# KMASAHIRO/AVR

Hardware: AMD Instinct MI355X
Metric: ray-samples/sec/GPU (1024 rays×256 samp×512 freq) + IR render ms/pose (higher is better)
Workload: dtype f32; 1 GPU; c2_meshrir_1024x256x512; mode=pose, rays=1024, samples=256, T=1022, freq_bins=512, distinct_poses=16, parallelism=poses x1 (no data-path collective)

## Files before the change

avr_amd/csrc/hashgrid.hip:

```cpp
#include "common.h"

#include <algorithm>

using namespace avr;

namespace {

constexpr int kMaxLevels = 32;

struct LevelTable {
    int64_t offset[kMaxLevels + 1];
    float scale[kMaxLevels];
    uint32_t res[kMaxLevels];
};

__device__ __forceinline__ uint32_t grid_index(uint32_t size, uint32_t res, uint32_t x, uint32_t y,
                                               uint32_t z) {
    uint64_t stride = 1;
    uint32_t index = 0;
    const uint32_t c[3] = {x, y, z};
#pragma unroll
    for (int d = 0; d < 3; ++d) {
        if (stride > size) break;
        index += c[d] * (uint32_t)stride;
        stride *= res;
    }
    if (size < stride) index = (x * 1u) ^ (y * 2654435761u) ^ (z * 805459861u);
    return index % size;
}

template <typename Tp>
__device__ __forceinline__ float2 load_pair(const Tp* params, int64_t entry);
template <>
__device__ __forceinline__ float2 load_pair<float>(const float* params, int64_t entry) {
    return *reinterpret_cast<const float2*>(params + 2 * entry);
}
template <>
__device__ __forceinline__ float2 load_pair<__half>(const __half* params, int64_t entry) {
    return __half22float2(*reinterpret_cast<const __half2*>(params + 2 * entry));
}

template <typename Tp>
struct CornerAcc;
template <>
struct CornerAcc<float> {
    using raw = float2;
    float2 a = make_float2(0.0f, 0.0f);
    __device__ __forceinline__ static raw load(const float* table, uint32_t e) {
        return *reinterpret_cast<const float2*>(table + 2 * (size_t)e);
    }
    __device__ __forceinline__ void add(float w, raw v) {
        a.x = fmaf(w, v.x, a.x);
        a.y = fmaf(w, v.y, a.y);
    }
    __device__ __forceinline__ float2 get() const { return a; }
};
template <>
struct CornerAcc<__half> {
    using raw = __half2;
    __half2 a = __float2half2_rn(0.0f);
    __device__ __forceinline__ static raw load(const __half* table, uint32_t e) {
        return *reinterpret_cast<const __half2*>(table + 2 * (size_t)e);
    }
    __device__ __forceinline__ void add(float w, raw v) {
        const __half2 w2 = __float2half2_rn(w);
        uint32_t r, wu, vu, au;
        __builtin_memcpy(&wu, &w2, 4);
        __builtin_memcpy(&vu, &v, 4);
        __builtin_memcpy(&au, &a, 4);
        asm("v_pk_fma_f16 %0, %1, %2, %3" : "=v"(r) : "v"(wu), "v"(vu), "v"(au));
        __builtin_memcpy(&a, &r, 4);
    }
    __device__ __forceinline__ float2 get() const { return __half22float2(a); }
};

template <typename To>
__device__ __forceinline__ void store_pair(To* out, int64_t i, float2 v);
template <>
__device__ __forceinline__ void store_pair<float>(float* out, int64_t i, float2 v) {
    *reinterpret_cast<float2*>(out + 2 * i) = v;
}
template <>
__device__ __forceinline__ void store_pair<__half>(__half* out, int64_t i, float2 v) {
    *reinterpret_cast<__half2*>(out + 2 * i) = __floats2half2_rn(v.x, v.y);
}

constexpr int64_t kLevelMajorMinPoints = 16384;
inline int64_t lm_min_points() { return kLevelMajorMinPoints; }

inline bool group_loads() { return true; }

struct Corner {
    float pos[3];
    uint32_t grid[3];
};

__device__ __forceinline__ Corner locate(const float* x, float scale) {
    Corner c;
#pragma unroll
    for (int d = 0; d < 3; ++d) {
        const float p = fmaf(scale, x[d], 0.5f);
        const float fl = floorf(p);
        c.grid[d] = (uint32_t)(int)fl;
        c.pos[d] = p - fl;
    }
    return c;
}

template <typename Tp, typename To>
__global__ __launch_bounds__(256) void hashgrid_fwd_kernel(int64_t N, int L,
                                                           const float* __restrict__ x,
                                                           const Tp* __restrict__ params,
                                                           LevelTable lt, To* __restrict__ out) {
    const int64_t q = (int64_t)blockIdx.x * blockDim.x + threadIdx.x;
    if (q >= N * L) return;
    const int64_t i = q / L;
    const int l = (int)(q % L);
    const float xi[3] = {x[i * 3 + 0], x[i * 3 + 1], x[i * 3 + 2]};
    const Corner c = locate(xi, lt.scale[l]);
    const uint32_t size = (uint32_t)(lt.offset[l + 1] - lt.offset[l]);
    const uint32_t res = lt.res[l];
    const Tp* table = params + 2 * lt.offset[l];
    CornerAcc<Tp> acc;
#pragma unroll
    for (int k = 0; k < 8; ++k) {
        float wgt = 1.0f;
        uint32_t g[3];
#pragma unroll
        for (int d = 0; d < 3; ++d) {
            if (k & (1 << d)) {
                wgt *= c.pos[d];
                g[d] = c.grid[d] + 1;
            } else {
                wgt *= 1.0f - c.pos[d];
                g[d] = c.grid[d];
            }
        }
        acc.add(wgt, CornerAcc<Tp>::load(table, grid_index(size, res, g[0], g[1], g[2])));
    }
    store_pair(out, q, acc.get());
}

template <typename Tp>
struct EntryGroup;
template <>
struct EntryGroup<__half> {
    static constexpr uint32_t kN = 4;
    uint32_t d[4];
    __device__ __forceinline__ void load(const __half* table, uint32_t e) {
        const uint4 v = *reinterpret_cast<const uint4*>(table + 2 * (e & ~(kN - 1)));
        d[0] = v.x;
        d[1] = v.y;
        d[2] = v.z;
        d[3] = v.w;
    }
    __device__ __forceinline__ __half2 get(uint32_t e) const {
        const uint32_t j = e & (kN - 1);
        const uint32_t v = j == 0 ? d[0] : j == 1 ? d[1] : j == 2 ? d[2] : d[3];
        __half2 h;
        __builtin_memcpy(&h, &v, 4);
        return h;
    }
};

template <typename Tp, typename To, bool ROW_MAJOR = false, bool GROUP = false>
__global__ __launch_bounds__(256) void hashgrid_fwd_lm_kernel(int64_t N, const float* __restrict__ x,
                                                              const Tp* __restrict__ params,
                                                              LevelTable lt, To* __restrict__ out, int unit) {
    const int l = blockIdx.y;
    const int64_t i = (int64_t)blockIdx.x * 256 + threadIdx.x;
    if (i >= N) return;
    float xi[3] = {x[i * 3 + 0], x[i * 3 + 1], x[i * 3 + 2]};
    if (unit) {
#pragma unroll
        for (int d = 0; d < 3; ++d) xi[d] = 0.5f + 0.5f * xi[d];
    }
    const Corner c = locate(xi, lt.scale[l]);
    const uint32_t size = (uint32_t)(lt.offset[l + 1] - lt.offset[l]);
    const uint32_t res = lt.res[l];
    const Tp* table = params + 2 * lt.offset[l];
    CornerAcc<Tp> acc;
    float wgt[8];
    uint32_t ent[8];
#pragma unroll
    for (int k = 0; k < 8; ++k) {
        float w = 1.0f;
        uint32_t g[3];
#pragma unroll
        for (int d = 0; d < 3; ++d) {
            if (k & (1 << d)) {
                w *= c.pos[d];
                g[d] = c.grid[d] + 1;
            } else {
                w *= 1.0f - c.pos[d];
                g[d] = c.grid[d];
            }
        }
        wgt[k] = w;
        ent[k] = grid_index(size, res, g[0], g[1], g[2]);
    }
    if constexpr (GROUP) {
        constexpr uint32_t kN = EntryGroup<Tp>::kN;
        EntryGroup<Tp> grp[4];
#pragma unroll
        for (int j = 0; j < 4; ++j) grp[j].load(table, ent[2 * j]);
        using raw = typename CornerAcc<Tp>::raw;
        raw far[4];
#pragma unroll
        for (int j = 0; j < 4; ++j) {
            far[j] = grp[j].get(ent[2 * j]);
            if ((ent[2 * j + 1] ^ ent[2 * j]) >= kN) far[j] = CornerAcc<Tp>::load(table, ent[2 * j + 1]);
        }
#pragma unroll
        for (int j = 0; j < 4; ++j) {
            const raw v0 = grp[j].get(ent[2 * j]);
            const raw v1 = ((ent[2 * j + 1] ^ ent[2 * j]) >= kN) ? far[j] : grp[j].get(ent[2 * j + 1]);
            acc.add(wgt[2 * j], v0);
            acc.add(wgt[2 * j + 1], v1);
        }
    } else {
#pragma unroll
        for (int k = 0; k < 8; ++k) acc.add(wgt[k], CornerAcc<Tp>::load(table, ent[k]));
    }
    store_pair(out, ROW_MAJOR ? i * (int64_t)gridDim.y + l : (int64_t)l * N + i, acc.get());
}

template <typename Tg, int RUN>
__global__ __launch_bounds__(256) void hashgrid_bwd_kernel(int64_t N, int L, int l0,
                                                           const float* __restrict__ x,
                                                           const Tg* __restrict__ gout,
                                                           LevelTable lt,
                                                           float* __restrict__ gparams) {
    const int l = l0 + (int)blockIdx.y;
    const int slot = threadIdx.x & 15;
    const int k = slot >> 1, f = slot & 1;
    const int64_t first = ((int64_t)blockIdx.x * 16 + (threadIdx.x >> 4)) * RUN;
    const uint32_t size = (uint32_t)(lt.offset[l + 1] - lt.offset[l]);
    const uint32_t res = lt.res[l];
    const float scale = lt.scale[l];
    float* __restrict__ table = gparams + 2 * lt.offset[l];
    float xi[RUN][3], g[RUN];
#pragma unroll
    for (int it = 0; it < RUN; ++it) {
        const int64_t i = first + it;
        const int64_t ic = i < N ? i : N - 1;
#pragma unroll
        for (int d = 0; d < 3; ++d) xi[it][d] = x[ic * 3 + d];
        g[it] = i < N ? load_f(gout, ic * (2 * L) + 2 * l + f) : 0.0f;
    }
    uint32_t pe = 0xffffffffu;
    float pv = 0.0f;
#pragma unroll
    for (int it = 0; it < RUN; ++it) {
        const Corner c = locate(xi[it], scale);
        float wgt = 1.0f;
        uint32_t gg[3];
#pragma unroll
        for (int d = 0; d < 3; ++d) {
            if (k & (1 << d)) {
                wgt *= c.pos[d];
                gg[d] = c.grid[d] + 1;
            } else {
                wgt *= 1.0f - c.pos[d];
                gg[d] = c.grid[d];
            }
        }
        const uint32_t e = 2u * grid_index(size, res, gg[0], gg[1], gg[2]) + (uint32_t)f;
        const float v = wgt * g[it];
        if (e == pe) {
            pv += v;
        } else {
            if (pv != 0.0f) atomicAdd(table + pe, pv);
            pe = e;
            pv = v;
        }
    }
    if (pv != 0.0f) atomicAdd(table + pe, pv);
}

inline int bwd_run() { return 16; }

template <typename Tg>
void launch_bwd(hipStream_t st, int64_t N, int L, const float* x, const Tg* gout, const LevelTable& lt,
                float* gparams) {
    const int run = bwd_run();
    const int64_t pts_per_block = 16 * (int64_t)run;
    const dim3 grid((unsigned)((N + pts_per_block - 1) / pts_per_block), (unsigned)L);
#define AVR_HG_BWD(I)                                                                                          \
    if (run == I) {                                                                                            \
        hipLaunchKernelGGL((hashgrid_bwd_kernel<Tg, I>), grid, dim3(256), 0, st, N, L, 0, x, gout, lt, gparams); \
        return;                                                                                                \
    }
    AVR_HG_BWD(1) AVR_HG_BWD(4) AVR_HG_BWD(8) AVR_HG_BWD(16) AVR_HG_BWD(32)
#undef AVR_HG_BWD
}

int make_table(int L, const int64_t* off, const float* scale, const int32_t* res, LevelTable* lt) {
    if (L < 1 || L > kMaxLevels) return fail(AVR_E_ARG, "hashgrid: n_levels out of range (1..32)");
    for (int l = 0; l <= L; ++l) lt->offset[l] = off[l];
    for (int l = 0; l < L; ++l) {
        lt->scale[l] = scale[l];
        lt->res[l] = (uint32_t)res[l];
        if (off[l + 1] <= off[l]) return fail(AVR_E_ARG, "hashgrid: empty level");
    }
    return 0;
}

template <typename Tp, typename To, bool ROW_MAJOR>
void launch_lm(dim3 grid, hipStream_t st, int64_t N, const float* x, const void* params, LevelTable lt,
               void* out, bool grp, int unit) {
    if constexpr (std::is_same_v<Tp, __half>) {
        if (grp) {
            hipLaunchKernelGGL((hashgrid_fwd_lm_kernel<Tp, To, ROW_MAJOR, true>), grid, dim3(256), 0, st, N,
                               x, (const Tp*)params, lt, (To*)out, unit);
            return;
        }
    }
    hipLaunchKernelGGL((hashgrid_fwd_lm_kernel<Tp, To, ROW_MAJOR, false>), grid, dim3(256), 0, st, N, x,
                           (const Tp*)params, lt, (To*)out, unit);
}

template <bool ROW_MAJOR>
int launch_fwd_lm(dim3 grid, hipStream_t st, int64_t N, const float* x, const void* params,
                  int32_t param_dtype, const LevelTable& lt, void* out, int32_t out_dtype, int unit = 0) {
    const bool grp = group_loads() && ((uintptr_t)params & 15) == 0;
    if (param_dtype == AVR_DTYPE_F32 && out_dtype == AVR_DTYPE_F32)
        launch_lm<float, float, ROW_MAJOR>(grid, st, N, x, params, lt, out, grp, unit);
    else if (param_dtype == AVR_DTYPE_F32 && out_dtype == AVR_DTYPE_F16)
        launch_lm<float, __half, ROW_MAJOR>(grid, st, N, x, params, lt, out, grp, unit);
    else if (param_dtype == AVR_DTYPE_F16 && out_dtype == AVR_DTYPE_F16)
        launch_lm<__half, __half, ROW_MAJOR>(grid, st, N, x, params, lt, out, grp, unit);
    else if (param_dtype == AVR_DTYPE_F16 && out_dtype == AVR_DTYPE_F32)
        launch_lm<__half, float, ROW_MAJOR>(grid, st, N, x, params, lt, out, grp, unit);
    else
        return fail(AVR_E_ARG, "avr_hashgrid_fwd: unknown dtype");
    return 0;
}

constexpr int kPartBits = 10;
constexpr int kPartEntries = 1 << kPartBits;
constexpr int kBwdGroups = 32;
constexpr int kBwdRun = 16;
constexpr int kChunkPts = kBwdGroups * kBwdRun;
constexpr int kReduceWaves = 4;
constexpr int kMaxScatterParts = 4096;

struct BwdPlan {
    int pbase[kMaxLevels + 1];
    int nchunks;
    int max_parts;
    int slice_cap[kMaxLevels];
    int hot_above[kMaxLevels];
};

__device__ __forceinline__ void corner_value(const float (&xi)[3], float g0, float g1, int k, float scale,
                                             uint32_t size, uint32_t res, uint32_t& e, float& v0, float& v1) {
    const Corner c = locate(xi, scale);
    float wgt = 1.0f;
    uint32_t gg[3];
#pragma unroll
    for (int d = 0; d < 3; ++d) {
        if (k & (1 << d)) {
            wgt *= c.pos[d];
            gg[d] = c.grid[d] + 1;
        } else {
            wgt *= 1.0f - c.pos[d];
            gg[d] = c.grid[d];
        }
    }
    e = grid_index(size, res, gg[0], gg[1], gg[2]);
    v0 = wgt * g0;
    v1 = wgt * g1;
}

__device__ __forceinline__ int64_t glm_index(int64_t i, int64_t N, int l) { return ((int64_t)l * N + i) * 2; }

template <typename Tg>
__device__ __forceinline__ void point_inputs(int64_t i, int64_t N, int L, int l, const float* __restrict__ x,
                                             const Tg* __restrict__ glm, float (&xi)[3], float& g0, float& g1) {
    const bool live = i < N;
    const int64_t ic = live ? i : N - 1;
#pragma unroll
    for (int d = 0; d < 3; ++d) xi[d] = x[ic * 3 + d];
    const int64_t gi = glm_index(ic, N, l);
    g0 = live ? load_f(glm, gi) : 0.0f;
    g1 = live ? load_f(glm, gi + 1) : 0.0f;
}

template <typename Tg>
__global__ __launch_bounds__(256) void hg_level_major_kernel(int64_t N, int L, const Tg* __restrict__ in,
                                                             Tg* __restrict__ out) {
    extern __shared__ __attribute__((aligned(16))) char lm_s[];
    Tg* t = reinterpret_cast<Tg*>(lm_s);
    const int64_t i0 = (int64_t)blockIdx.x * 64;
    const int np = (int)min((int64_t)64, N - i0);
    const int W = 2 * L;
    for (int j = threadIdx.x; j < np * W; j += 256) t[j] = in[i0 * W + j];
    __syncthreads();
    for (int j = threadIdx.x; j < L * np * 2; j += 256) {
        const int l = j / (np * 2), r = j - l * (np * 2);
        out[((int64_t)l * N + i0) * 2 + r] = t[(r >> 1) * W + 2 * l + (r & 1)];
    }
}

template <typename Tg, class Emit>
__device__ __forceinline__ void bwd_walk(int64_t N, int L, int l, const float* __restrict__ x,
                                         const Tg* __restrict__ gout, const LevelTable& lt, Emit&& emit) {
    const int k = threadIdx.x & 7;
    const int64_t first = ((int64_t)blockIdx.x * kBwdGroups + (threadIdx.x >> 3)) * kBwdRun;
    const uint32_t size = (uint32_t)(lt.offset[l + 1] - lt.offset[l]);
    const uint32_t res = lt.res[l];
    const float scale = lt.scale[l];
    float xi[kBwdRun][3], g0[kBwdRun], g1[kBwdRun];
#pragma unroll
    for (int it = 0; it < kBwdRun; ++it) point_inputs(first + it, N, L, l, x, gout, xi[it], g0[it], g1[it]);
    uint32_t pe = 0xffffffffu;
    float p0 = 0.0f, p1 = 0.0f;
#pragma unroll
    for (int it = 0; it < kBwdRun; ++it) {
        uint32_t e;
        float v0, v1;
        corner_value(xi[it], g0[it], g1[it], k, scale, size, res, e, v0, v1);
        if (e == pe) {
            p0 += v0;
            p1 += v1;
        } else {
            if (pe != 0xffffffffu && (p0 != 0.0f || p1 != 0.0f)) emit(pe, p0, p1);
            pe = e;
            p0 = v0;
            p1 = v1;
        }
    }
    if (pe != 0xffffffffu && (p0 != 0.0f || p1 != 0.0f)) emit(pe, p0, p1);
}

template <typename Tg>
__global__ __launch_bounds__(256) void hg_bwd_count_kernel(int64_t N, int L, const float* __restrict__ x,
                                                           const Tg* __restrict__ gout, LevelTable lt,
                                                           BwdPlan plan, int* __restrict__ counts) {
    extern __shared__ int cnt_l[];
    const int l = blockIdx.y;
    const int P = plan.pbase[l + 1] - plan.pbase[l];
    for (int p = threadIdx.x; p < P; p += 256) cnt_l[p] = 0;
    __syncthreads();
    bwd_walk(N, L, l, x, gout, lt,
             [&](uint32_t e, float, float) { atomicAdd(&cnt_l[e >> kPartBits], 1); });
    __syncthreads();
    for (int p = threadIdx.x; p < P; p += 256)
        counts[(int64_t)(plan.pbase[l] + p) * plan.nchunks + blockIdx.x] = cnt_l[p];
}

__global__ __launch_bounds__(1024) void hg_bwd_scan_kernel(int total_parts, int nchunks, int* __restrict__ counts,
                                                           int* __restrict__ totals) {
    const int lane = threadIdx.x & 63;
    const int p = blockIdx.x * 16 + (threadIdx.x >> 6);
    if (p >= total_parts) return;
    int* c = counts + (int64_t)p * nchunks;
    int carry = 0;
    for (int c0 = 0; c0 < nchunks; c0 += 64) {
        const int v = c0 + lane < nchunks ? c[c0 + lane] : 0;
        int incl = v;
#pragma unroll
        for (int off = 1; off < 64; off <<= 1) {
            const int o = __shfl_up(incl, off, 64);
            if (lane >= off) incl += o;
        }
        if (c0 + lane < nchunks) c[c0 + lane] = carry + incl - v;
        carry += __shfl(incl, 63, 64);
    }
    if (lane == 0) totals[p] = carry;
}

constexpr int kDenseSlice = 1024;
constexpr int kTagRounds = 4;
constexpr int kHashedSlice = 16384;

__global__ __launch_bounds__(1024) void hg_bwd_plan_kernel(int total_parts, BwdPlan plan,
                                                           const int* __restrict__ totals,
                                                           int* __restrict__ part_start,
                                                           int* __restrict__ slice_base) {
    __shared__ int ws_t[16], ws_s[16];
    __shared__ int pbase_s[kMaxLevels + 1], hot_s[kMaxLevels], cap_s[kMaxLevels];
    const int lane = threadIdx.x & 63, wave = threadIdx.x >> 6;
    if (threadIdx.x <= kMaxLevels) pbase_s[threadIdx.x] = plan.pbase[threadIdx.x];
    if (threadIdx.x < kMaxLevels) {
        hot_s[threadIdx.x] = plan.hot_above[threadIdx.x];
        cap_s[threadIdx.x] = plan.slice_cap[threadIdx.x];
    }
    __syncthreads();
    const int per = (total_parts + 1 + 1023) / 1024;
    const int q0 = threadIdx.x * per;
    int l0 = 0;
    while (l0 < kMaxLevels && pbase_s[l0 + 1] <= q0) ++l0;
    auto slices = [&](int t, int l) {
        const int cap = t > hot_s[l] ? kDenseSlice : cap_s[l];
        return max(1, (t + cap - 1) / cap);
    };
    int st = 0, ss = 0;
    int l = l0;
    for (int j0 = 0; j0 < per; j0 += 8) {
        int tv[8];
#pragma unroll
        for (int u = 0; u < 8; ++u) {
            const int q = q0 + j0 + u;
            tv[u] = (j0 + u < per && q < total_parts) ? totals[q] : -1;
        }
#pragma unroll
        for (int u = 0; u < 8; ++u) {
            if (tv[u] < 0) break;
            const int q = q0 + j0 + u;
            while (pbase_s[l + 1] <= q) ++l;
            st += tv[u];
            ss += slices(tv[u], l);
        }
    }
    int it = st, is = ss;
#pragma unroll
    for (int off = 1; off < 64; off <<= 1) {
        const int ut = __shfl_up(it, off, 64), us = __shfl_up(is, off, 64);
        if (lane >= off) {
            it += ut;
            is += us;
        }
    }
    if (lane == 63) {
        ws_t[wave] = it;
        ws_s[wave] = is;
    }
    __syncthreads();
    int pt = 0, ps = 0;
    for (int w = 0; w < wave; ++w) {
        pt += ws_t[w];
        ps += ws_s[w];
    }
    int rt = pt + it - st, rs = ps + is - ss;
    l = l0;
    for (int j0 = 0; j0 < per; j0 += 8) {
        int tv[8];
#pragma unroll
        for (int u = 0; u < 8; ++u) {
            const int q = q0 + j0 + u;
            tv[u] = (j0 + u < per && q < total_parts) ? totals[q] : -1;
        }
#pragma unroll
        for (int u = 0; u < 8; ++u) {
            const int q = q0 + j0 + u;
            if (j0 + u >= per || q > total_parts) break;
            part_start[q] = rt;
            slice_base[q] = rs;
            if (q == total_parts) break;
            while (pbase_s[l + 1] <= q) ++l;
            rt += tv[u];
            rs += slices(tv[u], l);
        }
    }
}

constexpr int kScatMaxRecs = 256 * kBwdRun;
static_assert(((int64_t)kMaxScatterParts << kPartBits) <= (int64_t(1) << 32), "staged key: partition + entry in 32 bits");
static_assert((3 * kScatMaxRecs + 3 * kMaxScatterParts + 1) * 4 + 16 <= 160 * 1024, "scatter LDS");

template <typename Tg>
__global__ __launch_bounds__(256) void hg_bwd_scatter_kernel(int64_t N, int L, const float* __restrict__ x,
                                                             const Tg* __restrict__ gout, LevelTable lt,
                                                             BwdPlan plan, const int* __restrict__ offs,
                                                             const int* __restrict__ totals,
                                                             const int* __restrict__ part_start,
                                                             uint3* __restrict__ contrib) {
    extern __shared__ __attribute__((aligned(16))) int scat_l[];
    __shared__ int wsum[4];
    const int l = blockIdx.y;
    const int pb = plan.pbase[l];
    const int P = plan.pbase[l + 1] - pb;
    uint32_t* stage = reinterpret_cast<uint32_t*>(scat_l);
    int* base = scat_l + 3 * kScatMaxRecs;
    int* lofs = base + P;
    int* slot = lofs + P + 1;
    const int chunk = blockIdx.x, nch = plan.nchunks;
    const int lane = threadIdx.x & 63, wave = threadIdx.x >> 6;
    const int E = (P + 255) / 256;
    const int q0 = threadIdx.x * E;
    int run = 0;
    for (int j = 0; j < E; ++j) {
        const int q = q0 + j;
        if (q >= P) break;
        const int64_t at = (int64_t)(pb + q) * nch + chunk;
// ... 177 lines not shown

struct BwdLayout {
    BwdPlan plan;
    int total_parts;
    int64_t counts, totals, part_start, slice_base, glm, contrib, bytes;
    int max_slices;
    bool scatter_ok;
};

int bwd_layout(int64_t N, int L, const int64_t* off, const int32_t* res, BwdLayout* o) {
    if (L < 1 || L > kMaxLevels) return fail(AVR_E_ARG, "hashgrid: n_levels out of range (1..32)");
    BwdLayout b{};
    bool res_dense[kMaxLevels];
    for (int l = 0; l < L; ++l) {
        const double cells = res ? (double)res[l] * res[l] * res[l] : 1e300;
        res_dense[l] = cells <= (double)(off[l + 1] - off[l]);
    }
    b.plan.pbase[0] = 0;
    b.plan.max_parts = 0;
    for (int l = 0; l < L; ++l) {
        const int64_t size = off[l + 1] - off[l];
        if (size <= 0 || size % 8) return fail(AVR_E_ARG, "hashgrid: level sizes must be positive multiples of 8");
        const int64_t P = (size + kPartEntries - 1) / kPartEntries;
        if (b.plan.pbase[l] + P > (1 << 24)) return fail(AVR_E_ARG, "hashgrid: tables too large");
        b.plan.pbase[l + 1] = b.plan.pbase[l] + (int)P;
        b.plan.slice_cap[l] = res_dense[l] ? kDenseSlice : kHashedSlice;
        const double share = (double)N * 8.0 * (double)std::min<int64_t>(size, kPartEntries) / (double)size;
        b.plan.hot_above[l] = res_dense[l] ? 0 : (int)std::min(1.5 * share + 64.0, 2.0e9);
        b.plan.max_parts = std::max(b.plan.max_parts, (int)P);
    }
    const int64_t nchunks = (N + kChunkPts - 1) / kChunkPts;
    const int64_t maxc = N * L * 8;
    if (maxc >= (int64_t(1) << 31) || nchunks > 65535)
        return fail(AVR_E_ARG, "hashgrid: too many points for the partitioned backward");
    b.plan.nchunks = (int)std::max<int64_t>(nchunks, 1);
    b.total_parts = b.plan.pbase[L];
    auto al = [](int64_t v) { return (v + 255) & ~(int64_t)255; };
    int64_t o0 = 0;
    b.counts = o0;
    o0 += al((int64_t)b.total_parts * b.plan.nchunks * 4);
    b.totals = o0;
    o0 += al((int64_t)b.total_parts * 4);
    b.part_start = o0;
    o0 += al((int64_t)(b.total_parts + 1) * 4);
    b.slice_base = o0;
    o0 += al((int64_t)(b.total_parts + 1) * 4);
    b.max_slices = b.total_parts + (int)(maxc / kDenseSlice) + 1;
    b.scatter_ok = b.plan.max_parts <= kMaxScatterParts;
    b.glm = o0;
    o0 += al(N * L * 2 * 4);
    b.contrib = o0;
    o0 += al(maxc * 12);
    b.bytes = o0;
    if (b.bytes > kMaxBwdWorkspaceBytes) b.scatter_ok = false;
    *o = b;
    return 0;
}

}

extern "C" int avr_hashgrid_fwd(int64_t N, int32_t n_levels, const float* x, const void* params,
                                int32_t param_dtype, const int64_t* level_offset,
                                const float* level_scale, const int32_t* level_res, void* out,
                                int32_t out_dtype, void* stream) {
    AVR_REQUIRE(N >= 0 && x && params && level_offset && level_scale && level_res && out,
                "avr_hashgrid_fwd: bad args");
    if (N == 0) return 0;
    LevelTable lt;
    if (int e = make_table(n_levels, level_offset, level_scale, level_res, &lt)) return e;
    const int64_t work = N * n_levels;
    const dim3 grid((unsigned)((work + 255) / 256));
    hipStream_t st = as_stream(stream);
    const int L = n_levels;
    if (N >= lm_min_points()) {
        const dim3 glm((unsigned)((N + 255) / 256), (unsigned)L);
        if (int e = launch_fwd_lm<true>(glm, st, N, x, params, param_dtype, lt, out, out_dtype)) return e;
        return check_launch("avr_hashgrid_fwd");
    }
    if (param_dtype == AVR_DTYPE_F32 && out_dtype == AVR_DTYPE_F32)
        hipLaunchKernelGGL((hashgrid_fwd_kernel<float, float>), grid, dim3(256), 0, st, N, L, x,
                           (const float*)params, lt, (float*)out);
    else if (param_dtype == AVR_DTYPE_F32 && out_dtype == AVR_DTYPE_F16)
        hipLaunchKernelGGL((hashgrid_fwd_kernel<float, __half>), grid, dim3(256), 0, st, N, L, x,
                           (const float*)params, lt, (__half*)out);
    else if (param_dtype == AVR_DTYPE_F16 && out_dtype == AVR_DTYPE_F16)
        hipLaunchKernelGGL((hashgrid_fwd_kernel<__half, __half>), grid, dim3(256), 0, st, N, L, x,
                           (const __half*)params, lt, (__half*)out);
    else if (param_dtype == AVR_DTYPE_F16 && out_dtype == AVR_DTYPE_F32)
        hipLaunchKernelGGL((hashgrid_fwd_kernel<__half, float>), grid, dim3(256), 0, st, N, L, x,
                           (const __half*)params, lt, (float*)out);
    else
        return fail(AVR_E_ARG, "avr_hashgrid_fwd: unknown dtype");
    return check_launch("avr_hashgrid_fwd");
}

extern "C" int avr_hashgrid_bwd(int64_t N, int32_t n_levels, const float* x, const void* grad_out,
                                int32_t grad_dtype, const int64_t* level_offset,
                                const float* level_scale, const int32_t* level_res,
                                float* grad_params, void* stream) {
    AVR_REQUIRE(N >= 0 && x && grad_out && level_offset && level_scale && level_res && grad_params,
                "avr_hashgrid_bwd: bad args");
    if (N == 0) return 0;
    LevelTable lt;
    if (int e = make_table(n_levels, level_offset, level_scale, level_res, &lt)) return e;
    hipStream_t st = as_stream(stream);
    if (grad_dtype == AVR_DTYPE_F32)
        launch_bwd<float>(st, N, (int)n_levels, x, (const float*)grad_out, lt, grad_params);
    else if (grad_dtype == AVR_DTYPE_F16)
        launch_bwd<__half>(st, N, (int)n_levels, x, (const __half*)grad_out, lt, grad_params);
    else
        return fail(AVR_E_ARG, "avr_hashgrid_bwd: unknown grad dtype");
    return check_launch("avr_hashgrid_bwd");
}

namespace {
int fwd_lm(int64_t N, int32_t n_levels, const float* x, const void* params, int32_t param_dtype,
           const int64_t* level_offset, const float* level_scale, const int32_t* level_res, void* out,
           int32_t out_dtype, void* stream, int unit) {
    AVR_REQUIRE(N >= 0 && x && params && level_offset && level_scale && level_res && out,
                "avr_hashgrid_fwd_lm: bad args");
    if (N == 0) return 0;
    LevelTable lt;
    if (int e = make_table(n_levels, level_offset, level_scale, level_res, &lt)) return e;
    const dim3 grid((unsigned)((N + 255) / 256), (unsigned)n_levels);
    hipStream_t st = as_stream(stream);
    if (int e = launch_fwd_lm<false>(grid, st, N, x, params, param_dtype, lt, out, out_dtype, unit)) return e;
    return check_launch("avr_hashgrid_fwd_lm");
}
}

extern "C" int avr_hashgrid_fwd_lm(int64_t N, int32_t n_levels, const float* x, const void* params,
                                   int32_t param_dtype, const int64_t* level_offset,
                                   const float* level_scale, const int32_t* level_res, void* out,
                                   int32_t out_dtype, void* stream) {
    return fwd_lm(N, n_levels, x, params, param_dtype, level_offset, level_scale, level_res, out, out_dtype, stream,
                  0);
}

extern "C" int avr_hashgrid_fwd_lm_unit(int64_t N, int32_t n_levels, const float* x, const void* params,
                                        int32_t param_dtype, const int64_t* level_offset,
                                        const float* level_scale, const int32_t* level_res, void* out,
                                        int32_t out_dtype, void* stream) {
    return fwd_lm(N, n_levels, x, params, param_dtype, level_offset, level_scale, level_res, out, out_dtype, stream,
                  1);
}

namespace {

constexpr int kBiasRays = 4;

template <typename Tp>
__device__ __forceinline__ float2 encode_point_level(const float* xi, const Tp* params, const LevelTable& lt, int l) {
    const Corner c = locate(xi, lt.scale[l]);
    const uint32_t size = (uint32_t)(lt.offset[l + 1] - lt.offset[l]);
    const uint32_t res = lt.res[l];
    const Tp* table = params + 2 * lt.offset[l];
    CornerAcc<Tp> acc;
#pragma unroll
    for (int k = 0; k < 8; ++k) {
        float wgt = 1.0f;
        uint32_t g[3];
#pragma unroll
        for (int d = 0; d < 3; ++d) {
            if (k & (1 << d)) {
                wgt *= c.pos[d];
                g[d] = c.grid[d] + 1;
            } else {
                wgt *= 1.0f - c.pos[d];
                g[d] = c.grid[d];
            }
        }
        acc.add(wgt, CornerAcc<Tp>::load(table, grid_index(size, res, g[0], g[1], g[2])));
    }
    return acc.get();
}

__device__ __forceinline__ float round_feature(float v, bool f16, bool mlp_f16) {
    if (f16) v = __half2float(__float2half(v));
    return mlp_f16 ? __half2float(__float2half(v))
                   : __bfloat162float(__float2bfloat16(v));
}

template <typename Tp>
__global__ __launch_bounds__(256) void ray_pose_bias_kernel(int B, int R, int S, const float* __restrict__ view,
                                                            const float* __restrict__ tx, const Tp* __restrict__ dp,
                                                            LevelTable dl, int dL, const Tp* __restrict__ tp,
                                                            LevelTable tl, int tL, int f16, int mlp_f16,
                                                            const float* __restrict__ wd,
                                                            const float* __restrict__ wt, int nout,
                                                            float* __restrict__ bias) {
    __shared__ float e[kBiasRays][2][2 * kMaxLevels];
    const int64_t g0 = (int64_t)blockIdx.x * kBiasRays;
    const int nr = (int)min((int64_t)kBiasRays, (int64_t)B * R - g0);
    for (int q = threadIdx.x; q < kBiasRays * 2 * kMaxLevels; q += 256) {
        const int j = q / (2 * kMaxLevels), rem = q % (2 * kMaxLevels);
        const int which = rem / kMaxLevels, l = rem % kMaxLevels;
        if (j >= nr || l >= (which ? tL : dL)) continue;
        const int64_t gr = g0 + j;
        const int64_t b = gr / R, r = gr % R;
        const float* src = which ? tx + b * R * S * 3 : view + (b * R * S + r * S) * 3;
        const float xi[3] = {(src[0] + 1.0f) / 2.0f, (src[1] + 1.0f) / 2.0f, (src[2] + 1.0f) / 2.0f};
        const float2 v = which ? encode_point_level(xi, tp, tl, l) : encode_point_level(xi, dp, dl, l);
        e[j][which][2 * l] = round_feature(v.x, f16, mlp_f16);
        e[j][which][2 * l + 1] = round_feature(v.y, f16, mlp_f16);
    }
    __syncthreads();
    auto skinny = [&](const float* __restrict__ w, int K2, int which, int o, float (&acc)[kBiasRays]) {
        int k = 0;
        for (; k + 8 <= K2; k += 8) {
            float wv[8];
#pragma unroll
            for (int u = 0; u < 8; ++u) wv[u] = w[(int64_t)(k + u) * nout + o];
#pragma unroll
            for (int u = 0; u < 8; ++u)
#pragma unroll
                for (int j = 0; j < kBiasRays; ++j) acc[j] = fmaf(e[j][which][k + u], wv[u], acc[j]);
        }
        for (; k < K2; ++k) {
            const float wv = w[(int64_t)k * nout + o];
#pragma unroll
            for (int j = 0; j < kBiasRays; ++j) acc[j] = fmaf(e[j][which][k], wv, acc[j]);
        }
    };
    for (int o = threadIdx.x; o < nout; o += 256) {
        float sd[kBiasRays], st[kBiasRays];
#pragma unroll
        for (int j = 0; j < kBiasRays; ++j) sd[j] = st[j] = 0.0f;
        skinny(wd, 2 * dL, 0, o, sd);
        skinny(wt, 2 * tL, 1, o, st);
#pragma unroll
        for (int j = 0; j < kBiasRays; ++j)
            if (j < nr) bias[(g0 + j) * nout + o] = sd[j] + st[j];
    }
}

constexpr int kBias2Rays = 4;
#ifndef AVR_BIAS_V1
#define AVR_BIAS_V1 0
#endif
constexpr int kBias2Threads = 512;

template <typename Tp>
__global__ __launch_bounds__(kBias2Threads) void ray_pose_bias2_kernel(
    int B, int R, int S, const float* __restrict__ view, const float* __restrict__ tx, const Tp* __restrict__ dp,
    LevelTable dl, int dL, const Tp* __restrict__ tp, LevelTable tl, int tL, int f16, int mlp_f16,
    const float* __restrict__ wd, const float* __restrict__ wt, int nout, float* __restrict__ bias) {
    __shared__ float ed[kBias2Rays][2 * kMaxLevels];
    __shared__ float et[2 * kMaxLevels];
    const int64_t g0 = (int64_t)blockIdx.x * kBias2Rays;
    const int64_t b = g0 / R;
    for (int q = threadIdx.x; q < (kBias2Rays + 1) * kMaxLevels; q += kBias2Threads) {
        const int j = q / kMaxLevels, l = q % kMaxLevels;
        const bool is_tx = j == kBias2Rays;
        if (l >= (is_tx ? tL : dL)) continue;
        const int64_t r = (g0 + j) % R;
        const float* src = is_tx ? tx + b * R * S * 3 : view + (b * R * S + r * S) * 3;
        const float xi[3] = {(src[0] + 1.0f) / 2.0f, (src[1] + 1.0f) / 2.0f, (src[2] + 1.0f) / 2.0f};
        const float2 v = is_tx ? encode_point_level(xi, tp, tl, l) : encode_point_level(xi, dp, dl, l);
        float* e = is_tx ? et : ed[j];
        e[2 * l] = round_feature(v.x, f16, mlp_f16);
        e[2 * l + 1] = round_feature(v.y, f16, mlp_f16);
    }
    __syncthreads();
    for (int o = threadIdx.x; o < nout; o += kBias2Threads) {
        constexpr int KB = 16;
        float st = 0.0f;
        for (int k0 = 0; k0 < 2 * tL; k0 += KB) {
            float w[KB];
#pragma unroll
            for (int u = 0; u < KB; ++u) w[u] = k0 + u < 2 * tL ? wt[(int64_t)(k0 + u) * nout + o] : 0.0f;
#pragma unroll
            for (int u = 0; u < KB; ++u)
                if (k0 + u < 2 * tL) st = fmaf(et[k0 + u], w[u], st);
        }
        float sd[kBias2Rays];
#pragma unroll
        for (int r = 0; r < kBias2Rays; ++r) sd[r] = 0.0f;
        for (int k0 = 0; k0 < 2 * dL; k0 += KB) {
            float w[KB];
#pragma unroll
            for (int u = 0; u < KB; ++u) w[u] = k0 + u < 2 * dL ? wd[(int64_t)(k0 + u) * nout + o] : 0.0f;
#pragma unroll
            for (int u = 0; u < KB; ++u)
                if (k0 + u < 2 * dL)
#pragma unroll
                    for (int r = 0; r < kBias2Rays; ++r) sd[r] = fmaf(ed[r][k0 + u], w[u], sd[r]);
        }
#pragma unroll
        for (int r = 0; r < kBias2Rays; ++r) bias[(g0 + r) * nout + o] = sd[r] + st;
    }
}

}

extern "C" int avr_ray_pose_bias(int32_t B, int32_t R, int32_t S, const float* view, const float* tx,
                                 int32_t dir_levels, const void* dir_params, const int64_t* dir_offset,
                                 const float* dir_scale, const int32_t* dir_res, int32_t tx_levels,
                                 const void* tx_params, const int64_t* tx_offset, const float* tx_scale,
                                 const int32_t* tx_res, int32_t param_dtype, int32_t enc_dtype,
                                 int32_t mlp_dtype, const float* w_dir, const float* w_tx, int32_t n_out,
                                 float* bias, void* stream) {
    AVR_REQUIRE(B >= 1 && R >= 1 && S >= 1 && view && tx && dir_params && tx_params && w_dir && w_tx && bias &&
                    n_out >= 1,
                "avr_ray_pose_bias: bad args");
    AVR_REQUIRE(enc_dtype == AVR_DTYPE_F16 || enc_dtype == AVR_DTYPE_F32, "avr_ray_pose_bias: enc dtype");
    AVR_REQUIRE(mlp_dtype == AVR_DTYPE_BF16 || mlp_dtype == AVR_DTYPE_F16, "avr_ray_pose_bias: mlp dtype");
    const int mlp_f16 = mlp_dtype == AVR_DTYPE_F16;
    LevelTable dl, tl;
    if (int e = make_table(dir_levels, dir_offset, dir_scale, dir_res, &dl)) return e;
    if (int e = make_table(tx_levels, tx_offset, tx_scale, tx_res, &tl)) return e;
    const int64_t rays = (int64_t)B * R;
    const dim3 grid((unsigned)((rays + kBiasRays - 1) / kBiasRays));
    const int f16 = enc_dtype == AVR_DTYPE_F16;
    hipStream_t st = as_stream(stream);
    if (R % kBias2Rays == 0 && !AVR_BIAS_V1) {
        const dim3 grid2((unsigned)(rays / kBias2Rays));
        if (param_dtype == AVR_DTYPE_F16)
            hipLaunchKernelGGL(ray_pose_bias2_kernel<__half>, grid2, dim3(kBias2Threads), 0, st, (int)B, (int)R,
                               (int)S, view, tx, (const __half*)dir_params, dl, (int)dir_levels,
                               (const __half*)tx_params, tl, (int)tx_levels, f16, mlp_f16, w_dir, w_tx, (int)n_out,
                               bias);
        else if (param_dtype == AVR_DTYPE_F32)
            hipLaunchKernelGGL(ray_pose_bias2_kernel<float>, grid2, dim3(kBias2Threads), 0, st, (int)B, (int)R,
                               (int)S, view, tx, (const float*)dir_params, dl, (int)dir_levels,
                               (const float*)tx_params, tl, (int)tx_levels, f16, mlp_f16, w_dir, w_tx, (int)n_out,
                               bias);
// ... 131 lines not shown
```

Before: 2.281 billion ray-samples/s.

## Specialize hash-grid corner indexing per level kind on the host

The host now classifies each hash-grid level as dense, power-of-two hashed, or generic and stores that kind in the level table. Kernels then compute the eight corner entries with specialized code: shared hash products and a mask instead of modulo for power-of-two tables, and a base offset plus strides for dense levels. The grouped half-precision path only issues the far loads when some pair crosses a group, and the per-entry selector becomes a two-level select. This cuts integer multiply and modulo work in the forward and backward encoders, at the cost of more code paths and a runtime branch per level kind.

```diff
diff --git a/avr_amd/csrc/hashgrid.hip b/avr_amd/csrc/hashgrid.hip
--- a/avr_amd/csrc/hashgrid.hip
+++ b/avr_amd/csrc/hashgrid.hip
@@ -1,4 +1,5 @@
 #include "common.h"
+#include "hashgrid_index.h"
 
 #include <algorithm>
 
@@ -12,21 +13,11 @@
     int64_t offset[kMaxLevels + 1];
     float scale[kMaxLevels];
     uint32_t res[kMaxLevels];
+    uint32_t kind[kMaxLevels];
 };
 
-__device__ __forceinline__ uint32_t grid_index(uint32_t size, uint32_t res, uint32_t x, uint32_t y,
-                                               uint32_t z) {
-    uint64_t stride = 1;
-    uint32_t index = 0;
-    const uint32_t c[3] = {x, y, z};
-#pragma unroll
-    for (int d = 0; d < 3; ++d) {
-        if (stride > size) break;
-        index += c[d] * (uint32_t)stride;
-        stride *= res;
-    }
-    if (size < stride) index = (x * 1u) ^ (y * 2654435761u) ^ (z * 805459861u);
-    return index % size;
+__device__ __forceinline__ LevelIndex level_of(const LevelTable& lt, int l) {
+    return level_index((uint32_t)(lt.offset[l + 1] - lt.offset[l]), lt.res[l], lt.kind[l]);
 }
 
 template <typename Tp>
@@ -105,6 +96,24 @@
         c.pos[d] = p - fl;
     }
     return c;
+}
+
+__device__ __forceinline__ void corner_weights(const Corner& c, float (&w)[8]) {
+    float a[3][2];
+#pragma unroll
+    for (int d = 0; d < 3; ++d) {
+        a[d][0] = 1.0f - c.pos[d];
+        a[d][1] = c.pos[d];
+    }
+#pragma unroll
+    for (int k = 0; k < 8; ++k) w[k] = (a[0][k & 1] * a[1][(k >> 1) & 1]) * a[2][k >> 2];
+}
+
+__device__ __forceinline__ float corner_weight(const Corner& c, int k) {
+    const float wx = (k & 1) ? c.pos[0] : 1.0f - c.pos[0];
+    const float wy = (k & 2) ? c.pos[1] : 1.0f - c.pos[1];
+    const float wz = (k & 4) ? c.pos[2] : 1.0f - c.pos[2];
+    return (wx * wy) * wz;
 }
 
 template <typename Tp, typename To>
@@ -118,26 +127,14 @@
     const int l = (int)(q % L);
     const float xi[3] = {x[i * 3 + 0], x[i * 3 + 1], x[i * 3 + 2]};
     const Corner c = locate(xi, lt.scale[l]);
-    const uint32_t size = (uint32_t)(lt.offset[l + 1] - lt.offset[l]);
-    const uint32_t res = lt.res[l];
     const Tp* table = params + 2 * lt.offset[l];
+    float wgt[8];
+    uint32_t ent[8];
+    corner_weights(c, wgt);
+    corner_entries(level_of(lt, l), c.grid, ent);
     CornerAcc<Tp> acc;
 #pragma unroll
-    for (int k = 0; k < 8; ++k) {
-        float wgt = 1.0f;
-        uint32_t g[3];
-#pragma unroll
-        for (int d = 0; d < 3; ++d) {
-            if (k & (1 << d)) {
-                wgt *= c.pos[d];
-                g[d] = c.grid[d] + 1;
-            } else {
-                wgt *= 1.0f - c.pos[d];
-                g[d] = c.grid[d];
-            }
-        }
-        acc.add(wgt, CornerAcc<Tp>::load(table, grid_index(size, res, g[0], g[1], g[2])));
-    }
+    for (int k = 0; k < 8; ++k) acc.add(wgt[k], CornerAcc<Tp>::load(table, ent[k]));
     store_pair(out, q, acc.get());
 }
 
@@ -155,8 +152,9 @@
         d[3] = v.w;
     }
     __device__ __forceinline__ __half2 get(uint32_t e) const {
-        const uint32_t j = e & (kN - 1);
-        const uint32_t v = j == 0 ? d[0] : j == 1 ? d[1] : j == 2 ? d[2] : d[3];
+        const bool hi = (e & 2u) != 0, odd = (e & 1u) != 0;
+        const uint32_t a = hi ? d[2] : d[0], b = hi ? d[3] : d[1];
+        const uint32_t v = odd ? b : a;
         __half2 h;
         __builtin_memcpy(&h, &v, 4);
         return h;
@@ -176,45 +174,35 @@
         for (int d = 0; d < 3; ++d) xi[d] = 0.5f + 0.5f * xi[d];
     }
     const Corner c = locate(xi, lt.scale[l]);
-    const uint32_t size = (uint32_t)(lt.offset[l + 1] - lt.offset[l]);
-    const uint32_t res = lt.res[l];
     const Tp* table = params + 2 * lt.offset[l];
     CornerAcc<Tp> acc;
     float wgt[8];
     uint32_t ent[8];
-#pragma unroll
-    for (int k = 0; k < 8; ++k) {
-        float w = 1.0f;
-        uint32_t g[3];
-#pragma unroll
-        for (int d = 0; d < 3; ++d) {
-            if (k & (1 << d)) {
-                w *= c.pos[d];
-                g[d] = c.grid[d] + 1;
-            } else {
-                w *= 1.0f - c.pos[d];
-                g[d] = c.grid[d];
-            }
-        }
-        wgt[k] = w;
-        ent[k] = grid_index(size, res, g[0], g[1], g[2]);
-    }
+    corner_weights(c, wgt);
+    corner_entries(level_of(lt, l), c.grid, ent);
     if constexpr (GROUP) {
         constexpr uint32_t kN = EntryGroup<Tp>::kN;
         EntryGroup<Tp> grp[4];
 #pragma unroll
         for (int j = 0; j < 4; ++j) grp[j].load(table, ent[2 * j]);
         using raw = typename CornerAcc<Tp>::raw;
-        raw far[4];
+        bool out_of_group[4];
+        bool any = false;
 #pragma unroll
         for (int j = 0; j < 4; ++j) {
-            far[j] = grp[j].get(ent[2 * j]);
-            if ((ent[2 * j + 1] ^ ent[2 * j]) >= kN) far[j] = CornerAcc<Tp>::load(table, ent[2 * j + 1]);
+            out_of_group[j] = (ent[2 * j + 1] ^ ent[2 * j]) >= kN;
+            any = any || out_of_group[j];
+        }
+        raw far[4] = {};
+        if (any) {
+#pragma unroll
+            for (int j = 0; j < 4; ++j) far[j] = CornerAcc<Tp>::load(table, ent[2 * j + 1]);
         }
 #pragma unroll
         for (int j = 0; j < 4; ++j) {
             const raw v0 = grp[j].get(ent[2 * j]);
-            const raw v1 = ((ent[2 * j + 1] ^ ent[2 * j]) >= kN) ? far[j] : grp[j].get(ent[2 * j + 1]);
+            const raw in_group = grp[j].get(ent[2 * j + 1]);
+            const raw v1 = out_of_group[j] ? far[j] : in_group;
             acc.add(wgt[2 * j], v0);
             acc.add(wgt[2 * j + 1], v1);
         }
@@ -235,8 +223,7 @@
     const int slot = threadIdx.x & 15;
     const int k = slot >> 1, f = slot & 1;
     const int64_t first = ((int64_t)blockIdx.x * 16 + (threadIdx.x >> 4)) * RUN;
-    const uint32_t size = (uint32_t)(lt.offset[l + 1] - lt.offset[l]);
-    const uint32_t res = lt.res[l];
+    const LevelIndex ix = level_of(lt, l);
     const float scale = lt.scale[l];
     float* __restrict__ table = gparams + 2 * lt.offset[l];
     float xi[RUN][3], g[RUN];
@@ -248,34 +235,27 @@
         for (int d = 0; d < 3; ++d) xi[it][d] = x[ic * 3 + d];
         g[it] = i < N ? load_f(gout, ic * (2 * L) + 2 * l + f) : 0.0f;
     }
-    uint32_t pe = 0xffffffffu;
-    float pv = 0.0f;
-#pragma unroll
-    for (int it = 0; it < RUN; ++it) {
-        const Corner c = locate(xi[it], scale);
-        float wgt = 1.0f;
-        uint32_t gg[3];
-#pragma unroll
-        for (int d = 0; d < 3; ++d) {
-            if (k & (1 << d)) {
-                wgt *= c.pos[d];
-                gg[d] = c.grid[d] + 1;
+    for_level_kind(ix.kind, [&](auto kind) {
+        uint32_t pe = 0xffffffffu;
+        float pv = 0.0f;
+#pragma unroll
+        for (int it = 0; it < RUN; ++it) {
+            const Corner c = locate(xi[it], scale);
+            const uint32_t e = 2u * corner_entry_of<decltype(kind)::value>(ix, c.grid[0] + (k & 1),
+                                                                           c.grid[1] + ((k >> 1) & 1),
+                                                                           c.grid[2] + (k >> 2)) +
+                               (uint32_t)f;
+            const float v = corner_weight(c, k) * g[it];
+            if (e == pe) {
+                pv += v;
             } else {
-                wgt *= 1.0f - c.pos[d];
-                gg[d] = c.grid[d];
+                if (pv != 0.0f) atomicAdd(table + pe, pv);
+                pe = e;
+                pv = v;
             }
         }
-        const uint32_t e = 2u * grid_index(size, res, gg[0], gg[1], gg[2]) + (uint32_t)f;
-        const float v = wgt * g[it];
-        if (e == pe) {
-            pv += v;
-        } else {
-            if (pv != 0.0f) atomicAdd(table + pe, pv);
-            pe = e;
-            pv = v;
-        }
-    }
-    if (pv != 0.0f) atomicAdd(table + pe, pv);
+        if (pv != 0.0f) atomicAdd(table + pe, pv);
+    });
 }
 
 inline int bwd_run() { return 16; }
@@ -302,6 +282,8 @@
         lt->scale[l] = scale[l];
         lt->res[l] = (uint32_t)res[l];
         if (off[l + 1] <= off[l]) return fail(AVR_E_ARG, "hashgrid: empty level");
+        if (off[l + 1] - off[l] > (int64_t)0xffffffffll) return fail(AVR_E_ARG, "hashgrid: level too large");
+        lt->kind[l] = classify_level((uint32_t)(off[l + 1] - off[l]), lt->res[l]);
     }
     return 0;
 }
@@ -353,22 +335,12 @@
     int hot_above[kMaxLevels];
 };
 
+template <uint32_t KIND>
 __device__ __forceinline__ void corner_value(const float (&xi)[3], float g0, float g1, int k, float scale,
-                                             uint32_t size, uint32_t res, uint32_t& e, float& v0, float& v1) {
+                                             const LevelIndex& ix, uint32_t& e, float& v0, float& v1) {
     const Corner c = locate(xi, scale);
-    float wgt = 1.0f;
-    uint32_t gg[3];
-#pragma unroll
-    for (int d = 0; d < 3; ++d) {
-        if (k & (1 << d)) {
-            wgt *= c.pos[d];
-            gg[d] = c.grid[d] + 1;
-        } else {
-            wgt *= 1.0f - c.pos[d];
-            gg[d] = c.grid[d];
-        }
-    }
-    e = grid_index(size, res, gg[0], gg[1], gg[2]);
+    const float wgt = corner_weight(c, k);
+    e = corner_entry_of<KIND>(ix, c.grid[0] + (k & 1), c.grid[1] + ((k >> 1) & 1), c.grid[2] + (k >> 2));
     v0 = wgt * g0;
     v1 = wgt * g1;
 }
@@ -408,30 +380,31 @@
                                          const Tg* __restrict__ gout, const LevelTable& lt, Emit&& emit) {
     const int k = threadIdx.x & 7;
     const int64_t first = ((int64_t)blockIdx.x * kBwdGroups + (threadIdx.x >> 3)) * kBwdRun;
-    const uint32_t size = (uint32_t)(lt.offset[l + 1] - lt.offset[l]);
-    const uint32_t res = lt.res[l];
+    const LevelIndex ix = level_of(lt, l);
     const float scale = lt.scale[l];
     float xi[kBwdRun][3], g0[kBwdRun], g1[kBwdRun];
 #pragma unroll
     for (int it = 0; it < kBwdRun; ++it) point_inputs(first + it, N, L, l, x, gout, xi[it], g0[it], g1[it]);
-    uint32_t pe = 0xffffffffu;
-    float p0 = 0.0f, p1 = 0.0f;
-#pragma unroll
-    for (int it = 0; it < kBwdRun; ++it) {
-        uint32_t e;
-        float v0, v1;
-        corner_value(xi[it], g0[it], g1[it], k, scale, size, res, e, v0, v1);
-        if (e == pe) {
-            p0 += v0;
-            p1 += v1;
-        } else {
-            if (pe != 0xffffffffu && (p0 != 0.0f || p1 != 0.0f)) emit(pe, p0, p1);
-            pe = e;
-            p0 = v0;
-            p1 = v1;
-        }
-    }
-    if (pe != 0xffffffffu && (p0 != 0.0f || p1 != 0.0f)) emit(pe, p0, p1);
+    for_level_kind(ix.kind, [&](auto kind) {
+        uint32_t pe = 0xffffffffu;
+        float p0 = 0.0f, p1 = 0.0f;
+#pragma unroll
+        for (int it = 0; it < kBwdRun; ++it) {
+            uint32_t e;
+            float v0, v1;
+            corner_value<decltype(kind)::value>(xi[it], g0[it], g1[it], k, scale, ix, e, v0, v1);
+            if (e == pe) {
+                p0 += v0;
+                p1 += v1;
+            } else {
+                if (pe != 0xffffffffu && (p0 != 0.0f || p1 != 0.0f)) emit(pe, p0, p1);
+                pe = e;
+                p0 = v0;
+                p1 = v1;
+            }
+        }
+        if (pe != 0xffffffffu && (p0 != 0.0f || p1 != 0.0f)) emit(pe, p0, p1);
+    });
 }
 
 template <typename Tg>
@@ -915,26 +888,14 @@
 template <typename Tp>
 __device__ __forceinline__ float2 encode_point_level(const float* xi, const Tp* params, const LevelTable& lt, int l) {
     const Corner c = locate(xi, lt.scale[l]);
-    const uint32_t size = (uint32_t)(lt.offset[l + 1] - lt.offset[l]);
-    const uint32_t res = lt.res[l];
     const Tp* table = params + 2 * lt.offset[l];
+    float wgt[8];
+    uint32_t ent[8];
+    corner_weights(c, wgt);
+    corner_entries(level_of(lt, l), c.grid, ent);
     CornerAcc<Tp> acc;
 #pragma unroll
-    for (int k = 0; k < 8; ++k) {
-        float wgt = 1.0f;
-        uint32_t g[3];
-#pragma unroll
-        for (int d = 0; d < 3; ++d) {
-            if (k & (1 << d)) {
-                wgt *= c.pos[d];
-                g[d] = c.grid[d] + 1;
-            } else {
-                wgt *= 1.0f - c.pos[d];
-                g[d] = c.grid[d];
-            }
-        }
-        acc.add(wgt, CornerAcc<Tp>::load(table, grid_index(size, res, g[0], g[1], g[2])));
-    }
+    for (int k = 0; k < 8; ++k) acc.add(wgt[k], CornerAcc<Tp>::load(table, ent[k]));
     return acc.get();
 }
 
diff --git a/avr_amd/csrc/hashgrid_index.h b/avr_amd/csrc/hashgrid_index.h
--- /dev/null
+++ b/avr_amd/csrc/hashgrid_index.h
@@ -0,0 +1,111 @@
+#pragma once
+
+#include <stdint.h>
+
+#if defined(__HIPCC__)
+#define AVR_HG_HD __host__ __device__ __forceinline__
+#define AVR_HG_UNROLL _Pragma("unroll")
+#else
+#define AVR_HG_HD inline
+#define AVR_HG_UNROLL
+#endif
+
+namespace avr {
+
+constexpr uint32_t kHashPrimeY = 2654435761u;
+constexpr uint32_t kHashPrimeZ = 805459861u;
+
+enum : uint32_t { kLevelGeneric = 0, kLevelHashedPow2 = 1, kLevelDense = 2 };
+template <uint32_t KIND>
+struct KindTag {
+    static constexpr uint32_t value = KIND;
+};
+
+AVR_HG_HD uint32_t grid_index(uint32_t size, uint32_t res, uint32_t x, uint32_t y, uint32_t z) {
+    uint64_t stride = 1;
+    uint32_t index = 0;
+    const uint32_t c[3] = {x, y, z};
+AVR_HG_UNROLL
+    for (int d = 0; d < 3; ++d) {
+        if (stride > size) break;
+        index += c[d] * (uint32_t)stride;
+        stride *= res;
+    }
+    if (size < stride) index = (x * 1u) ^ (y * kHashPrimeY) ^ (z * kHashPrimeZ);
+    return index % size;
+}
+
+AVR_HG_HD uint32_t classify_level(uint32_t size, uint32_t res) {
+    const uint64_t r = res;
+    const bool dense = r <= size && r * r <= size && r * r * r <= size;
+    if (dense) return res >= 1 ? kLevelDense : kLevelGeneric;
+    return (size & (size - 1)) == 0 ? kLevelHashedPow2 : kLevelGeneric;
+}
+
+struct LevelIndex {
+    uint32_t size, res, res2, kind;
+};
+
+AVR_HG_HD LevelIndex level_index(uint32_t size, uint32_t res, uint32_t kind) {
+    LevelIndex ix;
+    ix.size = size;
+    ix.res = res;
+    ix.res2 = res * res;
+    ix.kind = kind;
+    return ix;
+}
+
+AVR_HG_HD void corner_entries(const LevelIndex& ix, const uint32_t (&g)[3], uint32_t (&e)[8]) {
+    if (ix.kind == kLevelHashedPow2) {
+        const uint32_t mask = ix.size - 1;
+        const uint32_t xs[2] = {g[0], g[0] + 1};
+        uint32_t hy[2], hz[2];
+        hy[0] = g[1] * kHashPrimeY;
+        hy[1] = hy[0] + kHashPrimeY;
+        hz[0] = g[2] * kHashPrimeZ;
+        hz[1] = hz[0] + kHashPrimeZ;
+AVR_HG_UNROLL
+        for (int k = 0; k < 8; ++k) e[k] = (xs[k & 1] ^ (hy[(k >> 1) & 1] ^ hz[k >> 2])) & mask;
+    } else if (ix.kind == kLevelDense) {
+        const uint32_t base = g[0] + g[1] * ix.res + g[2] * ix.res2;
+AVR_HG_UNROLL
+        for (int k = 0; k < 8; ++k) e[k] = base + (k & 1) + ((k & 2) ? ix.res : 0u) + ((k & 4) ? ix.res2 : 0u);
+        const uint32_t lim = ix.res - 1;
+        if (!(g[0] < lim && g[1] < lim && g[2] < lim)) {
+AVR_HG_UNROLL
+            for (int k = 0; k < 8; ++k) e[k] %= ix.size;
+        }
+    } else {
+AVR_HG_UNROLL
+        for (int k = 0; k < 8; ++k)
+            e[k] = grid_index(ix.size, ix.res, g[0] + (k & 1), g[1] + ((k >> 1) & 1), g[2] + (k >> 2));
+    }
+}
+
+template <uint32_t KIND>
+AVR_HG_HD uint32_t corner_entry_of(const LevelIndex& ix, uint32_t x, uint32_t y, uint32_t z) {
+    if (KIND == kLevelHashedPow2) return (x ^ (y * kHashPrimeY) ^ (z * kHashPrimeZ)) & (ix.size - 1);
+    if (KIND == kLevelDense) {
+        const uint32_t e = x + y * ix.res + z * ix.res2;
+        return e >= ix.size ? e % ix.size : e;
+    }
+    return grid_index(ix.size, ix.res, x, y, z);
+}
+
+AVR_HG_HD uint32_t corner_entry(const LevelIndex& ix, uint32_t x, uint32_t y, uint32_t z) {
+    if (ix.kind == kLevelHashedPow2) return corner_entry_of<kLevelHashedPow2>(ix, x, y, z);
+    if (ix.kind == kLevelDense) return corner_entry_of<kLevelDense>(ix, x, y, z);
+    return corner_entry_of<kLevelGeneric>(ix, x, y, z);
+}
+
+template <class F>
+AVR_HG_HD void for_level_kind(uint32_t kind, F&& f) {
+    if (kind == kLevelHashedPow2)
+        f(KindTag<kLevelHashedPow2>{});
+    else if (kind == kLevelDense)
+        f(KindTag<kLevelDense>{});
+    else
+        f(KindTag<kLevelGeneric>{});
+}
+
+}
```

After: 2.277 billion ray-samples/s. Within noise of the previous version (-0.2%).
